# skywoodsz/qm_control

Hardware: NVIDIA H100
Metric: mpc_wbc_iters_per_s (higher is better)
Workload: dtype f64

## Files before the change

### qm_control_b200/csrc/kernels/mpc_api.cuh

```cuda
#pragma once
#include <cuda_runtime.h>

#include <string>
#include <vector>

#include "dev_common.cuh"

namespace qmb {

constexpr int EMAX = 32, KMAX = 4, TARGET_DIM = 37;
constexpr int LDX = 36, LDB = 28, LDG = 34, LDH = 24;
constexpr int ST_AR = 0;
constexpr int ST_BR = ST_AR + 9 * LDX;
constexpr int ST_Q = ST_BR + 9 * LDB;
constexpr int Q_PACKED = 480;
__host__ __device__ constexpr int q_row_offset(int r) { return (r & 1) ? 2 * ((r >> 1) + 1) * ((r >> 1) + 1) : 2 * (r >> 1) * ((r >> 1) + 1); }
__host__ __device__ constexpr int q_row_padded(int r) { return (r + 2) & ~1; }
static_assert(q_row_offset(29) + q_row_padded(29) == Q_PACKED && q_row_offset(1) == 2 && q_row_offset(2) == 4 && q_row_offset(3) == 8, "packed lower triangle with even rows");
constexpr int ST_TAIL = ST_Q + Q_PACKED;
constexpr int T_PXJ = 0;
constexpr int T_b = 144, T_q = 174, T_r = 204;
constexpr int T_RT = 222;
constexpr int T_SJ = 276;
constexpr int T_PU2 = 372, T_PED = 380;
constexpr int T_MISC = 396;
constexpr int T_INT = 400;
constexpr int TAIL_DBL = 428, STAGE_DBL = ST_TAIL + TAIL_DBL;
constexpr int SI_TYPE = 0, SI_M = 1, SI_NDEP = 2, SI_DEP = 3, SI_FREE = 19, SI_PIV = 37, SI_PCOL = 41;
static_assert(STAGE_DBL == 1484 && (ST_BR % 2 == 0) && (ST_Q % 2 == 0) && (ST_TAIL % 2 == 0) && (TAIL_DBL % 2 == 0), "16-byte aligned pieces");
constexpr int GAIN_DBL = 18 * LDG;
constexpr int ROBOT_DBL = 8;

struct MpcSolutionDev { int32_t* n_nodes = nullptr; double* t = nullptr; int32_t* event = nullptr; double* x = nullptr; double* u = nullptr; };

struct MpcBuffers {
  int B = 0, nmax = 0, cur = 0;
  double *t0 = nullptr, *x0 = nullptr, *event_times = nullptr, *target_times = nullptr, *target_states = nullptr;
  int32_t *n_events = nullptr, *modes = nullptr, *n_target = nullptr;
  MpcSolutionDev sol[2];
  double *ddp_trial = nullptr;
  double *node_rec = nullptr;
  double *stage = nullptr, *gains = nullptr, *dx = nullptr, *du = nullptr, *robot = nullptr, *step_info = nullptr;
  int32_t *stage_i = nullptr, *status = nullptr;
};
bool mpc_alloc(MpcBuffers& m, int B, int nmax, std::string& err, std::vector<void*>& allocs, cudaStream_t stream);
int mpc_configure_device();

struct MpcProblemDev { const double* t0; const double* x0; const int32_t* n_events; const double* event_times; const int32_t* modes; const int32_t* n_target; const double* target_times; const double* target_states;
                       const double* srbd; const double* tuning; };

int mpc_solve_launch(const DevModel* mdl, const DevModel& host_mdl, MpcBuffers& m, const MpcProblemDev& p, int b0, int b1, cudaStream_t stream, cudaEvent_t* ev = nullptr);
double measure_fp64_peak(cudaStream_t stream);
// ... 5 lines not shown
```

### qm_control_b200/csrc/kernels/mpc_kernels.cu

```cuda
#include <cstdlib>
#include "mpc_api.cuh"
#include "mpc_device.cuh"
#include "node_eval.cuh"
#include "wlinalg.cuh"

namespace qmb {

#ifndef QMB_LQ_WARPS
#define QMB_LQ_WARPS 4
#endif
#ifndef QMB_LQ_MINB
#define QMB_LQ_MINB 4
#endif
constexpr int LQ_WARPS = QMB_LQ_WARPS, LS_WARPS = 4, SETUP_WARPS = 4;
enum { MST_ITER_CAP = 1, MST_OVERFLOW = 2, MST_NAN = 4, MST_NOT_PD = 8, MST_NO_STEP = 16, MST_CONVERGED = 32, MST_NEG_DT = 64 };

__device__ __forceinline__ double interval_start(double t, int ev) { return ev == 2 ? t + WEAK_EPS : t; }
__device__ __forceinline__ double interval_end(double t, int ev) { return ev == 1 ? t - WEAK_EPS : t; }
__device__ __forceinline__ int clamp_events(int ne) { return ne < 0 ? 0 : (ne > EMAX ? EMAX : ne); }
__device__ __forceinline__ int clamp_targets(int nk) { return nk < 1 ? 1 : (nk > KMAX ? KMAX : nk); }
__device__ __forceinline__ int flag_mask(int mode) { int m = 0; for (int i = 0; i < 4; ++i) if (contact_flag(mode, i)) m |= 1 << i; return m; }

struct SetupIdx { int iu, ix; double au, ax; };
__host__ __device__ inline size_t setup_smem_per_warp(int nmax) { return (size_t)nmax * (8 + 8 + 4 + sizeof(SetupIdx) + 4) + 8 * EMAX + 64; }
__global__ void __launch_bounds__(32 * SETUP_WARPS) mpc_setup_kernel(const DevModel* __restrict__ mdl, int b0, int B, int nmax, MpcProblemDev p, MpcSolutionDev prev, MpcSolutionDev next, int32_t* __restrict__ status) {
  const int warp = threadIdx.x >> 5, lane = threadIdx.x & 31; const int b = b0 + blockIdx.x * SETUP_WARPS + warp; if (b >= B) return;
  extern __shared__ __align__(16) unsigned char s_setup[];
  unsigned char* base = s_setup + (size_t)warp * ((setup_smem_per_warp(nmax) + 15) & ~(size_t)15);
  double* spt = reinterpret_cast<double*>(base); double* sgt = spt + nmax; SetupIdx* sidx = reinterpret_cast<SetupIdx*>(sgt + nmax); double* sev = reinterpret_cast<double*>(sidx + nmax);
  int32_t* sge = reinterpret_cast<int32_t*>(sev + EMAX); int32_t* sflag = sge + nmax; unsigned char* smodes = reinterpret_cast<unsigned char*>(sflag + nmax);
  const double t0 = p.t0[b], tf = t0 + mdl->time_horizon, dt = mdl->dt; const int ne = clamp_events(p.n_events[b]); int st = 0;
  if (ne != p.n_events[b] || clamp_targets(p.n_target[b]) != p.n_target[b]) st |= MST_OVERFLOW;
  { const double* gev = p.event_times + (size_t)b * EMAX; const int32_t* gmodes = p.modes + (size_t)b * (EMAX + 1); sev[lane] = (lane < ne) ? gev[lane] : 0.0; smodes[lane] = (unsigned char)((lane <= ne) ? gmodes[lane] : 15); if (lane == 0) smodes[EMAX] = (unsigned char)((EMAX <= ne) ? gmodes[EMAX] : 15); }
  __syncwarp();
  const double* ev = sev; const unsigned char* modes = smodes;
// ... 36 lines not shown
  for (int k = 0; k < n - 1; ++k) {
    const int flag = sflag[k]; const SetupIdx ix = sidx[k]; double uk = 0.0;
    if (flag == 1) { uk = lerp(pu, ix.iu, ix.au); xk = lerp(px, ix.ix, ix.ax); }
    else if (flag == 0) { const int mode = ix.iu; int nst = 0; for (int i = 0; i < 4; ++i) nst += contact_flag(mode, i); if (lane < 12 && (lane % 3) == 2 && contact_flag(mode, lane / 3)) uk = srbd_of(mdl, p.srbd, b)->m * 9.81 / nst; }
    if (lane < NX) { gu[(size_t)k * NU + lane] = uk; gx[(size_t)(k + 1) * NX + lane] = xk; }
  }
  if (lane < NX && n >= 1) gu[(size_t)(n - 1) * NU + lane] = 0.0;
  if (lane == 0) status[b] = st;
}

struct LqLate { double BrdF[9 * 12], BrdJ[3 * NJ], bvec[NX]; };
struct alignas(16) LqSmem {
  ne::NodeRec rec;
  QuadWs quad; LegWs leg[4];
  double x[NX], u[NU];
  double Rw[NU][3];
  double Pe_full[NU], rs[NU];
  double ev[EMAX];
  int dep_idx[MAXDEP], free_idx[MU], col_of_input[NU];
  unsigned char modes[EMAX + 1];
};
static_assert(sizeof(LqLate) <= 4 * sizeof(ne::FootBlk) && offsetof(ne::NodeRec, foot) == 0, "LqLate overlays the foot blocks of the record");
static_assert(sizeof(LqSmem) % 16 == 0 && offsetof(LqSmem, rec) == 0, "aligned record slice");
static_assert((sizeof(LqSmem) * LQ_WARPS + 1024) * QMB_LQ_MINB <= 232448, "projection kernel: QMB_LQ_MINB CTAs of LQ_WARPS warps per SM (10.0 KB per node: four CTAs of four warps = 16 nodes in flight; 20 warps would fit the shared memory, not the 96-register budget)");

#ifndef QMB_FL_MINB
#define QMB_FL_MINB 2
#endif
constexpr int FL_WARPS = 4, FL_TILE = ne::EE_DBL;
constexpr int FL_UROW = NU + 1;
constexpr int FL_SMEM = FL_WARPS * 32 * (FL_TILE + 1 + FL_UROW) * 8;
__global__ void __launch_bounds__(32 * FL_WARPS, QMB_FL_MINB) mpc_flow_kernel(const DevModel* __restrict__ mdl, int b0, int B, int nmax, MpcProblemDev p, MpcSolutionDev sol, double* __restrict__ rec, const int32_t* __restrict__ status) {
  extern __shared__ __align__(16) unsigned char smem_raw[]; double (*tile)[32][FL_TILE + 1] = reinterpret_cast<double (*)[32][FL_TILE + 1]>(smem_raw);
  const int tid = threadIdx.x, warp = tid >> 5, lane = tid & 31; const long long gid = (long long)blockIdx.x * (32 * FL_WARPS) + tid;
  const int b = b0 + (int)(gid / nmax), k = (int)(gid % nmax);
  const int n = (b < B) ? sol.n_nodes[b] : 0;
  bool work = b < B && k < n && !(status[b] & MST_CONVERGED);
  const bool terminal = work && (k == n - 1);
  if (work && !terminal && sol.event[(size_t)b * nmax + k] == 1) work = false;
  const unsigned active = __ballot_sync(FULL, work); if (!active) return;
  const SrbdConst* sc = srbd_of(mdl, p.srbd, work ? b : b0);
  double* row = &tile[warp][lane][0]; double* gbase = rec + ((size_t)b0 * nmax + (size_t)(gid - lane)) * ne::NODE_REC_DBL;
  auto flush = [&](int off, int cnt) {
    __syncwarp();
#pragma unroll 4
    for (int rw = 0; rw < 32; ++rw) if ((active >> rw) & 1u) { double* g = gbase + (size_t)rw * ne::NODE_REC_DBL + off;
#pragma unroll
// ... 86 lines not shown
  if (!terminal && ek == 1) {
    double* tl = sg + ST_TAIL; int32_t* si = reinterpret_cast<int32_t*>(tl + T_INT);
    double d = 0.0; if (lane < NX) { d = xv - xnv; tl[T_b + lane] = d; }
    const double ss = warp_sum(d * d);
    if (lane == 0) { si[SI_TYPE] = 1; si[SI_M] = 0; si[SI_NDEP] = 0; tl[T_MISC] = 0.0; tl[T_MISC + 1] = 0.0; tl[T_MISC + 2] = ss; tl[T_MISC + 3] = 0.0; }
    return;
  }
  { double2* rs = reinterpret_cast<double2*>(&sm.rec);
#pragma unroll
    for (int q = 0; q < (ne::NODE_REC_DBL / 2 + 31) / 32; ++q) { const int e = lane + 32 * q; if (e < ne::NODE_REC_DBL / 2) rs[e] = rr[q]; } }
  __syncwarp();
  const int lfp = pack_leg_foot(mdl);
  const int nk = clamp_targets(p.n_target[b]); const double* tt = p.target_times + (size_t)b * KMAX; const double* ts = p.target_states + (size_t)b * KMAX * TARGET_DIM;
  const double t = interval_start(tk, ek);
  const double dt = terminal ? 0.0 : interval_end(tk1, ek1) - t;
  const int mode = mode_at_time(ev, modes, ne, t); const int fm = terminal ? 0 : flag_mask(mode);
  if (!terminal && !(dt > 0.0) && lane == 0) atomicOr(&status[b], MST_NEG_DT);
  double cost_val = 0.0, eq_ss = 0.0; int ndep = 0, m = 0; double b1v[3] = {0.0, 0.0, 0.0}, b2v[3] = {0.0, 0.0, 0.0}, a1[9], a2[9];
  {
  struct XU { double x[NX], u[NU]; }; static_assert(offsetof(LqSmem, u) == offsetof(LqSmem, x) + NX * 8, "x then u");
  cost_val = stage_cost_quad(mdl, sc, tuning_of(mdl, TUNED ? p.tuning : nullptr, b), reinterpret_cast<const XU*>(sm.x), &sm.rec.ee, &sm.quad, target_xnom(tt, ts, nk, t, lane), fm, terminal, lane);
  if (terminal) {
    double* tl = sg + ST_TAIL; int32_t* si = reinterpret_cast<int32_t*>(tl + T_INT);
    for (int r = 0; r < NX; ++r) { const int a = ee_pos(r); if (lane < q_row_padded(r)) { const int cc = (lane <= r) ? ee_pos(lane) : -1; sg[ST_Q + q_row_offset(r) + lane] = (a >= 0 && cc >= 0) ? sm.quad.E[a * 12 + cc] : 0.0; } }
    if (lane < NX) tl[T_q + lane] = sm.quad.qf[lane];
    if (lane == 0) { si[SI_TYPE] = 2; si[SI_M] = 0; si[SI_NDEP] = 0; tl[T_MISC] = 0.0; tl[T_MISC + 1] = cost_val; tl[T_MISC + 2] = 0.0; tl[T_MISC + 3] = 0.0; }
    return;
  }
  int nd_before = 0; for (int i = 0; i < 4; ++i) if (i < lane) nd_before += ((fm >> i) & 1) ? 3 : 4;
  ndep = 0; for (int i = 0; i < 4; ++i) ndep += ((fm >> i) & 1) ? 3 : 4;
  m = NU - ndep;
  for (int e = lane; e < NU * 3; e += 32) { const int i = e / 3, c = e - 3 * i; sm.Rw[i][c] = (i < 24) ? quad_R(mdl, &sm.quad, i, 3 * (i / 3) + c) : (c == 0 ? quad_R(mdl, &sm.quad, i, i) : 0.0); }
  bool swing_ok = true; int pivot = -1;
  if (lane < 4) {
    const int i = lane; const int first = mdl->foot_leg[i]; LegWs& L = sm.leg[i]; L.first = first; L.stance = (fm >> i) & 1;
    if (L.stance) { for (int j = 0; j < 3; ++j) { sm.dep_idx[nd_before + j] = 12 + first + j; L.dep[j] = 1; } L.pivot = -1; for (int a = 0; a < 3; ++a) eq_ss += sm.rec.foot[i].e[a] * sm.rec.foot[i].e[a]; }
    else {
      double zp, zv; swing_ok = swing_reference(mdl, ev, modes, ne, i, t, zp, zv);
      double ez = sm.rec.foot[i].e[2] - zv; if (mdl->position_error_gain != 0.0) ez += mdl->position_error_gain * (sm.rec.foot[i].pf[2] - zp);
      sm.rec.foot[i].e[2] = ez;
      for (int a = 0; a < 3; ++a) { sm.dep_idx[nd_before + a] = 3 * i + a; eq_ss += sm.u[3 * i + a] * sm.u[3 * i + a]; }
      eq_ss += ez * ez;
      double best = -1.0; for (int j = 0; j < 3; ++j) { const double a = fabs(sm.rec.foot[i].Jl[3 * j + 2]); if (a > best) { best = a; pivot = j; } }
      sm.dep_idx[nd_before + 3] = 12 + first + pivot; L.pivot = pivot; for (int j = 0; j < 3; ++j) L.dep[j] = (j == pivot);
    }
  }
  eq_ss = warp_sum(eq_ss);
// ... 86 lines not shown
        if (pos >= 0) { double acc = 0.0;
          for (int j = 0; j < 3; ++j) if (L.dep[j]) acc = fma(lt.BrdJ[rr * NJ + first + j], L.Px[j][pos], acc);
          v += acc; } }
      out[rr] = v;
    }
#pragma unroll
    for (int rr = 0; rr < 9; ++rr) { if (c == rr + 3) out[rr] += 1.0; sg[ST_AR + rr * LDX + c] = out[rr]; }
  } else if (lane == 31) {
#pragma unroll
    for (int rr = 0; rr < 9; ++rr) sg[ST_AR + rr * LDX + 31] = 0.0;
  }
  for (int e = lane; e < 36; e += 32) sg[ST_AR + (e >> 2) * LDX + 32 + (e & 3)] = 0.0;
  for (int e = lane; e < 144; e += 32) { const int j12 = e / 12, c = e - 12 * j12; const LegWs& L = sm.leg[foot_of_leg_joint(lfp, j12)]; const int j = j12 % 3; tl[T_PXJ + e] = L.dep[j] ? L.Px[j][c] : 0.0; }
  for (int e = lane; e < 9 * LDB; e += 32) {
    const int rr = e / LDB, a = e - rr * LDB; const int r = 3 + rr; double v = 0.0;
    if (a < m) { const int fa = sm.free_idx[a];
      if (fa < 12) v = lt.BrdF[rr * 12 + fa];
      else if (r < 6) { v = lt.BrdJ[rr * NJ + fa - 12];
        if (fa < 24) { const LegWs& L = sm.leg[foot_of_leg_joint(lfp, fa - 12)]; if (!L.stance) { const int jf = (fa - 12) % 3; v += lt.BrdJ[rr * NJ + L.first + L.pivot] * L.Pu2[jf > L.pivot ? jf - 1 : jf]; } } }
    }
    sg[ST_BR + e] = v;
  }
  if (lane < NX) {
    const int r = lane; double acc[NX];
    if (mdl->q_is_diag) { const double qrr = mdl->Qdiag[r];
#pragma unroll
      for (int c = 0; c < NX; ++c) acc[c] = (c == r) ? qrr : 0.0; }
    else {
#pragma unroll
      for (int c = 0; c < NX; ++c) acc[c] = mdl->Q[r * NX + c]; }
    double qv = sm.quad.qf[r];
    const int ea = ee_pos(r);
    if (ea >= 0) {
#pragma unroll
      for (int c = 0; c < 6; ++c) { acc[6 + c] += sm.quad.E[ea * 12 + c]; acc[24 + c] += sm.quad.E[ea * 12 + 6 + c]; }
    }
#pragma unroll
    for (int i = 0; i < 4; ++i) {
      const LegWs& L = sm.leg[i]; const int first = L.first;
      const int pr = (r < 6) ? r : ((r >= 9 && r < 12) ? r - 3 : ((r >= 12 + first && r < 15 + first) ? 9 + r - 12 - first : -1));
      if (pr >= 0) {
        double blk[12];
#pragma unroll
        for (int c = 0; c < 12; ++c) blk[c] = 0.0;
        double w3[3] = {0.0, 0.0, 0.0};
        for (int j = 0; j < 3; ++j) if (L.dep[j]) { const double pj = L.Px[j][pr]; qv = fma(pj, sm.rs[12 + first + j], qv);
#pragma unroll
          for (int a = 0; a < 3; ++a) w3[a] = fma(pj, sm.Rw[12 + first + j][a], w3[a]); }
        for (int a = 0; a < 3; ++a) if (L.dep[a]) { const double wa = w3[a];
#pragma unroll
          for (int c = 0; c < 12; ++c) blk[c] = fma(wa, L.Px[a][c], blk[c]); }
#pragma unroll
        for (int c = 0; c < 6; ++c) acc[c] += blk[c];
#pragma unroll
        for (int c = 0; c < 3; ++c) acc[9 + c] += blk[6 + c];
#pragma unroll
        for (int l = 0; l < 4; ++l) if (first == 3 * l) {
#pragma unroll
          for (int c = 0; c < 3; ++c) acc[12 + 3 * l + c] += blk[9 + c]; }
      }
    }
    const double dq = sm.quad.qdiag[r];
#pragma unroll
    for (int c = 0; c < NX; ++c) if (r <= c) sg[ST_Q + q_row_offset(c) + r] = dt * (acc[c] + ((c == r) ? dq : 0.0));
    if (!(r & 1)) sg[ST_Q + q_row_offset(r) + r + 1] = 0.0;
    tl[T_q + r] = dt * qv;
  }
  for (int e = lane; e < 8 * 12; e += 32) tl[T_SJ + e] = 0.0;
  __syncwarp();
  if (lane < MU) {
    const int a = lane; double rt[3] = {0.0, 0.0, 0.0}; double rtil = 0.0;
    if (a < m) {
      const int fa = sm.free_idx[a]; double rv = sm.rs[fa]; int li = -1, jf = -1;
      if (fa >= 12 && fa < 24) { li = foot_of_leg_joint(lfp, fa - 12); jf = (fa - 12) % 3; }
      const bool swing_joint = li >= 0 && !sm.leg[li].stance;
      const double* Rl = sm.Rw[jf >= 0 ? fa - jf : 0];
      if (swing_joint) {
        const LegWs& L = sm.leg[li]; const int pv = L.pivot; const int jfi = jf > pv ? jf - 1 : jf; const double pu = L.Pu2[jfi];
        rv += pu * sm.rs[fa - jf + pv];
        const double coef = Rl[3 * jf + pv]; double* Srow = tl + T_SJ + (2 * li + jfi) * 12;
        const double cf = dt * (coef + pu * Rl[3 * pv + pv]);
        for (int c = 0; c < 12; ++c) Srow[c] = cf * L.Px[pv][c];
      }
      rtil = dt * rv;
      if (fa >= 24) rt[0] = dt * sm.Rw[fa][0];
      else { const int bi = fa / 3;
        for (int jc = 0; jc < 3; ++jc) { const int fc = 3 * bi + jc; if (sm.col_of_input[fc] < 0) continue;
          double v = sm.Rw[fa][jc];
          if (swing_joint) { const LegWs& L = sm.leg[li]; const int pv = L.pivot; const double pa = L.Pu2[jf > pv ? jf - 1 : jf], pc = L.Pu2[jc > pv ? jc - 1 : jc];
            v += pa * Rl[3 * pv + jc] + Rl[3 * jf + pv] * pc + pa * Rl[3 * pv + pv] * pc; }
          rt[jc] = dt * v; } }
    }
    tl[T_r + a] = rtil; tl[T_RT + 3 * a] = rt[0]; tl[T_RT + 3 * a + 1] = rt[1]; tl[T_RT + 3 * a + 2] = rt[2];
  }
  if (lane < 4) { const LegWs& L = sm.leg[lane]; tl[T_PU2 + 2 * lane] = L.Pu2[0]; tl[T_PU2 + 2 * lane + 1] = L.Pu2[1]; si[SI_PIV + lane] = L.stance ? -1 : L.pivot;
    int nf = 0; for (int jj = 0; jj < 3; ++jj) if (!L.stance && jj != L.pivot) si[SI_PCOL + 2 * lane + nf++] = L.free_col[jj]; if (L.stance) { si[SI_PCOL + 2 * lane] = -1; si[SI_PCOL + 2 * lane + 1] = -1; } }
  if (lane < MAXDEP) { const int d = lane; double pe = 0.0; int di = -1; if (d < ndep) { di = sm.dep_idx[d]; pe = sm.Pe_full[di]; } tl[T_PED + d] = pe; si[SI_DEP + d] = di; }
  if (lane < MU) si[SI_FREE + lane] = (lane < m) ? sm.free_idx[lane] : -1;
  if (lane == 0) { si[SI_TYPE] = 0; si[SI_M] = m; si[SI_NDEP] = ndep; tl[T_MISC] = dtw; tl[T_MISC + 1] = dt * cost_val; tl[T_MISC + 2] = dt * dyn_ss; tl[T_MISC + 3] = dt * eq_ss; }
}

#ifndef QMB_TMA
#define QMB_TMA 1
#endif
constexpr int RIC_THREADS = 128, RIC_NTYPE = 512;
struct RicSmem {
  double P[NX * LDX];
  double A[NX * LDX];
  double W[NX * LDX];
  double Bm[NX * LDB], PB[NX * LDB];
  double G[MU * LDG];
  double H[MU * LDH];
  double Lt[MU * MU];
  alignas(16) double tail[TAIL_DBL];
  double dx[32], dut[32], tmp[32];
  double red[RIC_THREADS / 32][4];
  alignas(8) unsigned long long bar[4];
  int flag; int pad_;
  signed char srow[MU + 2], sfirst[MU + 2];
  unsigned char ntype[RIC_NTYPE];
};
static_assert(sizeof(RicSmem) <= 57344 - 64, "Riccati kernel must keep four CTAs per SM");

__device__ __forceinline__ unsigned smem_u32(const void* p) { return (unsigned)__cvta_generic_to_shared(p); }
__device__ __forceinline__ void mbar_init(unsigned long long* b, unsigned count) { asm volatile("mbarrier.init.shared::cta.b64 [%0], %1;\n" ::"r"(smem_u32(b)), "r"(count) : "memory"); }
__device__ __forceinline__ void mbar_expect_tx(unsigned long long* b, unsigned bytes) { asm volatile("mbarrier.arrive.expect_tx.shared::cta.b64 _, [%0], %1;\n" ::"r"(smem_u32(b)), "r"(bytes) : "memory"); }
__device__ __forceinline__ void mbar_wait(unsigned long long* b, unsigned parity) {
  asm volatile("{\n .reg .pred p;\n WAIT_LOOP:\n mbarrier.try_wait.parity.shared::cta.b64 p, [%0], %1;\n @p bra WAIT_DONE;\n bra WAIT_LOOP;\n WAIT_DONE:\n}\n" ::"r"(smem_u32(b)), "r"(parity) : "memory");
}
__device__ __forceinline__ void bulk_g2s(void* dst, const void* src, unsigned bytes, unsigned long long* bar) {
  asm volatile("cp.async.bulk.shared::cluster.global.mbarrier::complete_tx::bytes [%0], [%1], %2, [%3];\n" ::"r"(smem_u32(dst)), "l"(src), "r"(bytes), "r"(smem_u32(bar)) : "memory");
}
__device__ __forceinline__ int fresh_tid() { int t; asm volatile("mov.u32 %0, %%tid.x;" : "=r"(t)); return t; }
__device__ __forceinline__ void cp_async16(void* smem_dst, const void* gmem_src) { asm volatile("cp.async.cg.shared.global [%0], [%1], 16;\n" ::"r"(smem_u32(smem_dst)), "l"(gmem_src) : "memory"); }
__device__ __forceinline__ void cp_async_wait_all() { asm volatile("cp.async.wait_all;\n" ::: "memory"); }
struct CopyGroup {
  unsigned long long* bar; unsigned phase;
  __device__ __forceinline__ void begin(unsigned bytes, int tid) { if (QMB_TMA && tid == 0) mbar_expect_tx(bar, bytes); }
  __device__ __forceinline__ void copy(void* dst, const void* src, unsigned bytes, int tid, int nthr = RIC_THREADS, int t0 = 0) {
    if (QMB_TMA) { if (tid == 0) bulk_g2s(dst, src, bytes, bar); }
// ... 17 lines not shown
#pragma unroll
    for (int n = 0; n < NT; ++n) bf[n] = ok ? Y[kr * ldy + j0 + 8 * n + g] : 0.0;
#pragma unroll
    for (int m = 0; m < MT; ++m)
#pragma unroll
      for (int n = 0; n < NT; ++n) dmma884(c[m][n], a[m], bf[n]);
  }
}
template <int MT, int NT>
__device__ __forceinline__ void cfrag_load(const double* M, int ld, int i0, int j0, int rows, double (&c)[MT][NT][2], int g, int t) {
#pragma unroll
  for (int m = 0; m < MT; ++m)
#pragma unroll
    for (int n = 0; n < NT; ++n) { const int ri = i0 + 8 * m + g;
      if (ri < rows) { const double2 v = *reinterpret_cast<const double2*>(M + ri * ld + j0 + 8 * n + 2 * t); c[m][n][0] = v.x; c[m][n][1] = v.y; } else { c[m][n][0] = 0.0; c[m][n][1] = 0.0; } }
}
template <int MT, int NT>
__device__ __forceinline__ void cfrag_store(double* M, int ld, int i0, int j0, int rows, const double (&c)[MT][NT][2], int g, int t) {
#pragma unroll
  for (int m = 0; m < MT; ++m)
#pragma unroll
    for (int n = 0; n < NT; ++n) { const int ri = i0 + 8 * m + g; if (ri < rows) *reinterpret_cast<double2*>(M + ri * ld + j0 + 8 * n + 2 * t) = make_double2(c[m][n][0], c[m][n][1]); }
}
__device__ __forceinline__ int sup_pos(int j, int first) { return j < 6 ? j : ((j >= 9 && j < 12) ? j - 3 : (((unsigned)(j - 12 - first) < 3u) ? 9 + j - 12 - first : -1)); }

__global__ void __launch_bounds__(RIC_THREADS, 4) mpc_riccati_kernel(const DevModel* __restrict__ mdl, int b0, int B, int nmax, MpcProblemDev p, MpcSolutionDev sol, const double* __restrict__ stage,
                                                                  double* __restrict__ gains, double* __restrict__ dxo, double* __restrict__ duo, double* __restrict__ robot, int32_t* __restrict__ status) {
  extern __shared__ __align__(16) unsigned char smem_raw[];
  RicSmem& sm = *reinterpret_cast<RicSmem*>(smem_raw);
  const int tid = threadIdx.x, warp = tid >> 5, lane = tid & 31, ti = tid >> 2, jb = tid & 3; const int b = b0 + blockIdx.x;
  if (status[b] & MST_CONVERGED) return;
  const int n = sol.n_nodes[b]; const int N = n - 1;
  const double* sgb = stage + (size_t)b * nmax * STAGE_DBL; double* gb = gains + (size_t)b * nmax * GAIN_DBL;
  const int lfp = pack_leg_foot(mdl); const double imass = 1.0 / srbd_of(mdl, p.srbd, b)->m;
  for (int e = tid; e < (int)(sizeof(RicSmem) / 8); e += RIC_THREADS) reinterpret_cast<double*>(&sm)[e] = 0.0;
  __syncthreads();
  if (tid < NX && (tid < 3 || tid >= 24)) sm.A[tid * LDX + tid] = 1.0;
  if (tid == 0) { for (int i = 0; i < 4; ++i) mbar_init(&sm.bar[i], 1); asm volatile("fence.mbarrier_init.release.cluster;\n" ::: "memory"); }
  asm volatile("fence.proxy.async.shared::cta;\n" ::: "memory");
  const bool types_in_smem = n <= RIC_NTYPE;
  auto rec_type = [&](int k) -> int { return reinterpret_cast<const int32_t*>(sgb + (size_t)k * STAGE_DBL + ST_TAIL + T_INT)[SI_TYPE]; };
  if (types_in_smem) for (int k = tid; k < n; k += RIC_THREADS) sm.ntype[k] = (unsigned char)rec_type(k);
  auto node_type = [&](int k) -> int { return types_in_smem ? (int)sm.ntype[k] : rec_type(k); };
  CopyGroup gAB{&sm.bar[0], 0u}, gT{&sm.bar[1], 0u}, gQ{&sm.bar[2], 0u}, gF1{&sm.bar[3], 0u};
  auto issue_ab = [&](int k) { const double* sg = sgb + (size_t)k * STAGE_DBL; gAB.begin((9 * LDX + 9 * LDB) * 8, tid);
    gAB.copy(sm.A + 3 * LDX, sg + ST_AR, 9 * LDX * 8, tid); gAB.copy(sm.Bm + 3 * LDB, sg + ST_BR, 9 * LDB * 8, tid); };
  auto issue_tail = [&](int k) { gT.begin(TAIL_DBL * 8, tid); gT.copy(sm.tail, sgb + (size_t)k * STAGE_DBL + ST_TAIL, TAIL_DBL * 8, tid); };
  auto issue_q = [&](int k) { gQ.begin(Q_PACKED * 8, tid); gQ.copy(sm.Bm, sgb + (size_t)k * STAGE_DBL + ST_Q, Q_PACKED * 8, tid); };
  auto expand = [&]() { const int tid = fresh_tid();
    const double* tl = sm.tail; const int32_t* si = reinterpret_cast<const int32_t*>(tl + T_INT); const double dtw = tl[T_MISC];
    for (int e = tid; e < 144; e += RIC_THREADS) { const int j12 = e / 12, c = e - 12 * j12; const int col = sup_col(c, 3 * (j12 / 3));
      sm.A[(12 + j12) * LDX + col] = ((col == 12 + j12) ? 1.0 : 0.0) + dtw * tl[T_PXJ + e]; }
    if (tid < NX && (tid < 3 || tid >= 12)) sm.A[tid * LDX + NX] = tl[T_b + tid];
    for (int e = tid; e < 21 * MU; e += RIC_THREADS) {
      const int rr = e / MU, a = e - rr * MU; const int r = rr < 3 ? rr : rr + 9; const int fa = si[SI_FREE + a]; double v = 0.0;
      if (fa >= 0) {
        if (r < 3) { if (fa < 12 && fa - 3 * (fa / 3) == r) v = dtw * imass; }
        else if (fa == r) v = dtw;
        else if (fa >= 12 && fa < 24) { const int j = fa - 12, lg = j / 3, foot = (lfp >> (2 * lg)) & 3; const int pv = si[SI_PIV + foot];
          if (pv >= 0 && r == 12 + 3 * lg + pv) { const int jf = j - 3 * lg; v = dtw * tl[T_PU2 + 2 * foot + (jf > pv ? jf - 1 : jf)]; } }
      }
      sm.Bm[r * LDB + a] = v;
    }
    if (tid < MU) { const int fa = si[SI_FREE + tid]; int slot = -1, first = 0;
      if (fa >= 12 && fa < 24) { const int j = fa - 12, lg = j / 3, foot = (lfp >> (2 * lg)) & 3; const int pv = si[SI_PIV + foot]; if (pv >= 0) { const int jf = j - 3 * lg; slot = 2 * foot + (jf > pv ? jf - 1 : jf); first = 3 * lg; } }
      sm.srow[tid] = (signed char)slot; sm.sfirst[tid] = (signed char)first; }
  };
  for (int e = tid; e < NX * NX; e += RIC_THREADS) { const int r = e / NX, c = e - r * NX; sm.P[r * LDX + c] = sgb[(size_t)N * STAGE_DBL + ST_Q + q_row_offset(r > c ? r : c) + (r > c ? c : r)]; }
  if (tid < NX) sm.P[tid * LDX + NX] = sgb[(size_t)N * STAGE_DBL + ST_TAIL + T_q + tid];
  double perf0 = 0, perf1 = 0, perf2 = 0;
  for (int k = tid; k < n; k += RIC_THREADS) { const double* pf = sgb + (size_t)k * STAGE_DBL + ST_TAIL + T_MISC + 1; perf0 += pf[0]; perf1 += pf[1]; perf2 += pf[2]; }
  if (tid < NX) { const double d = p.x0[(size_t)b * NX + tid] - sol.x[(size_t)b * nmax * NX + tid]; sm.dx[tid] = d; perf1 += d * d; }
  perf0 = warp_sum(perf0); perf1 = warp_sum(perf1); perf2 = warp_sum(perf2);
  if (lane == 0) { sm.red[warp][0] = perf0; sm.red[warp][1] = perf1; sm.red[warp][2] = perf2; }
  __syncthreads();
  double perf[3]; for (int i = 0; i < 3; ++i) perf[i] = sm.red[0][i] + sm.red[1][i] + sm.red[2][i] + sm.red[3][i];
  if (N >= 1) { issue_tail(N - 1); if (node_type(N - 1) != 1) issue_ab(N - 1); gT.wait(); if (node_type(N - 1) != 1) expand(); }
  int st = 0;
  const int g = lane >> 2, t = lane & 3;
  for (int k = N - 1; k >= 0; --k) {
    const int type = node_type(k); const int tnext = k > 0 ? node_type(k - 1) : 1;
    if (type == 1) {
      __syncthreads();
      if (tid < NX) { double sv = sm.P[tid * LDX + NX]; for (int j = 0; j < NX; ++j) sv = fma(sm.P[tid * LDX + j], sm.tail[T_b + j], sv); sm.tmp[tid] = sv; }
      __syncthreads();
      if (tid < NX) sm.P[tid * LDX + NX] = sm.tmp[tid];
      if (k > 0) { issue_tail(k - 1); if (tnext != 1) issue_ab(k - 1); gT.wait(); if (tnext != 1) expand(); }
      continue;
    }
    gAB.wait(); if (QMB_TMA) __syncthreads();
    const double dtw_k = sm.tail[T_MISC]; const int acol0 = reinterpret_cast<const int32_t*>(sm.tail + T_INT)[SI_M] - 6;
// ... 20 lines not shown
    if (tid < NX) sm.P[tid * LDX + NX] = sm.tail[T_q + tid];
    { const double* tl = sm.tail; const int32_t* si = reinterpret_cast<const int32_t*>(tl + T_INT); const int mm = si[SI_M];
      double c[3][1][2];
#pragma unroll
      for (int mt = 0; mt < 3; ++mt) { const int a = 8 * mt + g; const bool rowok = a < MU; const int slot = rowok ? sm.srow[a] : -1, first = rowok ? sm.sfirst[a] : 0;
#pragma unroll
        for (int e = 0; e < 2; ++e) { const int j = 8 * warp + 2 * t + e; double v = 0.0;
          if (rowok) { if (j == NX) v = tl[T_r + a]; else if (slot >= 0 && j < NX) { const int ps = sup_pos(j, first); if (ps >= 0) v = tl[T_SJ + slot * 12 + ps]; }
            if ((unsigned)(a - acol0) < 6u) v = fma(dtw_k, sm.W[(24 + a - acol0) * LDX + j], v); }
          c[mt][0][e] = v; } }
      warp_mma<24, 3, 1, false>(sm.Bm, LDB, 0, sm.W, LDX, 8 * warp, c, g, t); cfrag_store<3, 1>(sm.G, LDG, 0, 8 * warp, MU, c, g, t);
      if (warp < 3) { double d[3][1][2];
#pragma unroll
        for (int mt = 0; mt < 3; ++mt) { const int a = 8 * mt + g; const int fa = (a < MU) ? si[SI_FREE + a] : -1;
#pragma unroll
          for (int e = 0; e < 2; ++e) { const int cc = 8 * warp + 2 * t + e; double v = 0.0;
            if (a < MU && cc < MU) { if (a >= mm) v = (a == cc) ? 1.0 : 0.0;
              else if (fa >= 24) v = (a == cc) ? tl[T_RT + 3 * a] : 0.0;
              else { const int fc = si[SI_FREE + cc]; if (fc >= 0 && fc / 3 == fa / 3) v = tl[T_RT + 3 * a + fc - 3 * (fc / 3)]; }
              if ((unsigned)(a - acol0) < 6u) v = fma(dtw_k, sm.PB[(24 + a - acol0) * LDB + cc], v); }
            d[mt][0][e] = v; } }
        warp_mma<24, 3, 1, false>(sm.Bm, LDB, 0, sm.PB, LDB, 8 * warp, d, g, t); cfrag_store<3, 1>(sm.H, LDH, 0, 8 * warp, MU, d, g, t); } }
    __syncthreads();
    issue_q(k);
    if (k > 0) issue_tail(k - 1);
    const int sw = (k + b) & 3;
    if (!QMB_TMA) gQ.wait();
    if (warp == sw) {
      if (QMB_TMA) gQ.skip();
      double hr[MU], y[MU]; double dinv = 0.0; bool ok = true; double* Yb = sm.PB;
#pragma unroll
      for (int c = 0; c < MU; ++c) { hr[c] = (lane < MU) ? sm.H[c * LDH + lane] : 0.0; y[c] = sm.G[c * LDG + lane]; }
#pragma unroll
      for (int j = 0; j < MU; ++j) {
        const double djj = __shfl_sync(FULL, hr[j], j); if (!(djj > 0.0)) ok = false;
        const double inv = rsqrt(djj); const double lij = hr[j] * inv;
        if (lane == j) dinv = inv;
        if (lane < MU) sm.Lt[j * MU + lane] = lij;
        y[j] *= inv; Yb[j * LDX + lane] = y[j];
#pragma unroll
        for (int c = j + 1; c < MU; ++c) { const double lcj = __shfl_sync(FULL, lij, c); hr[c] = fma(-lij, lcj, hr[c]); y[c] = fma(-lcj, y[j], y[c]); }
      }
      if (lane < MU) sm.dut[lane] = dinv;
      if (!ok && lane == 0) sm.flag = 1;
      __syncwarp();
      double* gk = gb + (size_t)k * GAIN_DBL;
#pragma unroll
      for (int a = MU - 1; a >= 0; --a) {
        asm volatile("" ::: "memory");
        y[a] *= sm.dut[a];
        gk[a * LDG + lane] = -y[a];
#pragma unroll
        for (int c = 0; c < a; ++c) y[c] = fma(-sm.Lt[c * MU + a], y[a], y[c]);
      }
    } else {
      if (QMB_TMA) gQ.wait();
      const int hi = (warp - sw - 1) & 3;
      for (int tile = hi; tile < 16; tile += 3) { const int i0 = 8 * (tile >> 2), j0 = 8 * (tile & 3);
        double c[1][1][2]; const int ri = i0 + g;
#pragma unroll
        for (int e = 0; e < 2; ++e) { const int cj = j0 + 2 * t + e; double v = (ri < NX && cj <= NX) ? (cj == NX ? sm.P[ri * LDX + NX] : (cj <= ri ? sm.Bm[q_row_offset(ri) + cj] : sm.Bm[q_row_offset(cj) + ri])) : 0.0;
          if (ri >= 24 && ri < NX && cj <= NX) v += sm.W[ri * LDX + cj];
          c[0][0][e] = v; }
        warp_mma<24, 1, 1, false>(sm.A, LDX, i0, sm.W, LDX, j0, c, g, t); cfrag_store<1, 1>(sm.P, LDX, i0, j0, NX, c, g, t); }
    }
    __syncthreads();
    if (sm.flag) { st |= MST_NOT_PD; if (k > 0) gT.wait(); break; }
    if (k > 0) { if (tnext != 1) issue_ab(k - 1); gT.wait(); if (tnext != 1) expand(); }
    { const double* Yb = sm.PB; const int i0 = 16 * (warp >> 1), j0 = 16 * (warp & 1);
      double c[2][2][2]; cfrag_load<2, 2>(sm.P, LDX, i0, j0, NX, c, g, t); warp_mma<MU, 2, 2, true>(Yb, LDX, i0, Yb, LDX, j0, c, g, t); cfrag_store<2, 2>(sm.P, LDX, i0, j0, NX, c, g, t); }
  }
  __syncthreads();
  double armijo = 0.0, dxn2 = 0.0, dun2 = 0.0;
  if (!(st & MST_NOT_PD)) {
    auto issue_fwd = [&](int k) {
      if (k >= N) return; const double* sg = sgb + (size_t)k * STAGE_DBL; const bool ev = node_type(k) == 1;
      auto issue = [&](CopyGroup& cg, double* kb, double* ab, double* bb) {
        cg.begin((ev ? 0 : (GAIN_DBL + 9 * LDX + 9 * LDB) * 8) + TAIL_DBL * 8, tid);
        cg.copy(ab + 9 * LDX, sg + ST_TAIL, TAIL_DBL * 8, tid);
        if (!ev) { cg.copy(kb, gb + (size_t)k * GAIN_DBL, GAIN_DBL * 8, tid); cg.copy(ab, sg + ST_AR, 9 * LDX * 8, tid); cg.copy(bb, sg + ST_BR, 9 * LDB * 8, tid); } };
      if (k & 1) issue(gF1, sm.W, sm.P, sm.PB); else issue(gAB, sm.G, sm.A, sm.Bm); };
    issue_fwd(0);
    for (int k = 0; k < N; ++k) {
      const int o = k & 1; const double* Kb = o ? sm.W : sm.G; const double* ARb = o ? sm.P : sm.A; const double* BRb = o ? sm.PB : sm.Bm; const double* tl = (o ? sm.P : sm.A) + 9 * LDX;
      double* dxk = dxo + ((size_t)b * nmax + k) * NX; double* duk = duo + ((size_t)b * nmax + k) * NU;
      const double* dxc = (k & 1) ? sm.tmp : sm.dx; double* dxn = (k & 1) ? sm.dx : sm.tmp;
// ... 394 lines not shown
```

### qm_control_b200/csrc/kernels/mpc_scalar.cuh

```cuda
#pragma once
#include "dev_common.cuh"

namespace qmb {

constexpr int MU = 18;
constexpr int MAXDEP = 16;
constexpr double WEAK_EPS = 1e-6;
QMB_HD int pack_leg_foot(const DevModel* __restrict__ mdl) { return mdl->leg_foot[0] | (mdl->leg_foot[1] << 2) | (mdl->leg_foot[2] << 4) | (mdl->leg_foot[3] << 6); }
QMB_HD int foot_of_leg_joint(int lfp, int j) { return (lfp >> (2 * (j / 3))) & 3; }
QMB_HD int lower_bound_idx(const double* a, int n, double t) { int lo = 0, hi = n; while (lo < hi) { const int mid = (lo + hi) >> 1; if (a[mid] < t) lo = mid + 1; else hi = mid; } return lo; }
template <class MT> QMB_HD int mode_at_time(const double* ev, const MT* modes, int ne, double t) { return modes[lower_bound_idx(ev, ne, t)]; }
QMB_HD void time_segment(const double* times, int n, double t, int& index, double& alpha) {
  if (n <= 1) { index = 0; alpha = 1.0; return; }
  const int part = lower_bound_idx(times, n, t); int idx = (part != 0 || t != times[0]) ? part - 1 : 0; const int last = n - 1;
  if (idx >= 0) {
    if (idx < last) { const double len = times[idx + 1] - times[idx], till = times[idx + 1] - t; index = idx; alpha = (len > 2.0 * 2.220446049250313e-16) ? till / len : (till > 0.5 * len ? 1.0 : 0.0); return; }
    index = (last - 1 > 0) ? last - 1 : 0; alpha = 0.0; return;
  }
  index = 0; alpha = 1.0;
}
template <class MT> QMB_HD bool swing_reference(const DevModel* __restrict__ mdl, const double* ev, const MT* modes, int ne, int leg, double t, double& zp, double& zv) {
  const int np = ne + 1; const int p = lower_bound_idx(ev, ne, t); zp = 0.0; zv = 0.0;
  if (contact_flag(modes[p], leg)) return true;
  int start = -1; for (int ip = p - 1; ip >= 0; --ip) if (contact_flag(modes[ip], leg)) { start = ip; break; }
  int fin = np - 1; for (int ip = p + 1; ip < np; ++ip) if (contact_flag(modes[ip], leg)) { fin = ip - 1; break; }
  if (start < 0 || fin >= np - 1) return false;
  const double t0 = ev[start], t1 = ev[fin]; const double scaling = fmin(1.0, (t1 - t0) / mdl->swing_time_scale); const double tm = 0.5 * (t0 + t1), zm = scaling * mdl->swing_height;
  double ta, pa, va, tb, pb, vb;
  if (t < tm) { ta = t0; pa = 0.0; va = scaling * mdl->lift_off_velocity; tb = tm; pb = zm; vb = 0.0; } else { ta = tm; pa = zm; va = 0.0; tb = t1; pb = 0.0; vb = scaling * mdl->touch_down_velocity; }
  const double dtt = tb - ta, dp = pb - pa, dv = vb - va; const double c0 = pa, c1 = va * dtt, c2 = -(3.0 * va + dv) * dtt + 3.0 * dp, c3 = (2.0 * va + dv) * dtt - 2.0 * dp; const double idt = 1.0 / dtt, tn = (t - ta) * idt;
  zp = ((c3 * tn + c2) * tn + c1) * tn + c0; zv = ((3.0 * c3 * tn + 2.0 * c2) * tn + c1) * idt; return true;
}
QMB_HD void relaxed_barrier(double mu, double delta, double h, double& p0, double& p1, double& p2) {
  const bool inside = h > delta; const double lg = log(inside ? h : delta);
  if (inside) { const double ih = 1.0 / h; p0 = -mu * lg; p1 = -mu * ih; p2 = mu * ih * ih; }
  else { const double t = (h - 2.0 * delta) / delta; p0 = mu * (-lg + 0.5 * t * t - 0.5); p1 = mu * (h - 2.0 * delta) / (delta * delta); p2 = mu / (delta * delta); }
}

QMB_HD int ee_pos(int c) { return (c >= 6 && c < 12) ? c - 6 : (c >= 24 ? c - 18 : -1); }
QMB_HD int ee_col(int i) { return i < 6 ? 6 + i : 18 + i; }
QMB_HD int sup_col(int pos, int first) { return pos < 6 ? pos : (pos < 9 ? pos + 3 : 12 + first + pos - 9); }

struct QuadWs { double E[144], fric[36], qdiag[NX], rdiag[NU], qf[NX], rf[NU]; };
QMB_HD double quad_R(const DevModel* __restrict__ mdl, const QuadWs* q, int i, int j) {
  if (i >= 24 || j >= 24) return (i == j) ? mdl->Rarm[i - 24] + q->rdiag[i] : 0.0;
  const int bi = i / 3; if (bi != j / 3) return 0.0;
  double v = mdl->Rblk[bi][(i - 3 * bi) * 3 + (j - 3 * bi)]; if (i == j) v += q->rdiag[i]; if (i < 12) v += q->fric[bi * 9 + (i - 3 * bi) * 3 + (j - 3 * bi)]; return v; }
struct LegWs {
  double Px[3][12];
  double G[9];
  double Pu2[2];
  int dep[3];
  int pivot, stance, first, free_col[3];
};

}
```

Measured before the change: 24.51.

## Store factored stage cost instead of packed dense Q and rebuild Q in Riccati

Replaces the packed 30x30 lower-triangle Q in each stage record with a compact cost block: the triangle of the 12x12 end-effector block, the diagonal, the leg Rw terms and a flag for a dense model Q. The Riccati kernel now pulls this block together with A/B in one TMA group and rebuilds Q on the fly, adding the leg projection term with an extra small MMA. This shrinks the stage record, removes the separate Q copy and its barrier, and drops the per-lane dense Q assembly from the LQ kernel. It also raises LQ occupancy (min blocks 5) and halves the node-type table. The cost is extra index arithmetic and a named barrier among three warps in the Riccati inner loop.

Result: faster. 24.94, median of 6 (+1.8%).

```diff
diff --git a/qm_control_b200/csrc/kernels/mpc_api.cuh b/qm_control_b200/csrc/kernels/mpc_api.cuh
--- a/qm_control_b200/csrc/kernels/mpc_api.cuh
+++ b/qm_control_b200/csrc/kernels/mpc_api.cuh
@@ -12,12 +12,15 @@
 constexpr int LDX = 36, LDB = 28, LDG = 34, LDH = 24;
 constexpr int ST_AR = 0;
 constexpr int ST_BR = ST_AR + 9 * LDX;
-constexpr int ST_Q = ST_BR + 9 * LDB;
-constexpr int Q_PACKED = 480;
-__host__ __device__ constexpr int q_row_offset(int r) { return (r & 1) ? 2 * ((r >> 1) + 1) * ((r >> 1) + 1) : 2 * (r >> 1) * ((r >> 1) + 1); }
-__host__ __device__ constexpr int q_row_padded(int r) { return (r + 2) & ~1; }
-static_assert(q_row_offset(29) + q_row_padded(29) == Q_PACKED && q_row_offset(1) == 2 && q_row_offset(2) == 4 && q_row_offset(3) == 8, "packed lower triangle with even rows");
-constexpr int ST_TAIL = ST_Q + Q_PACKED;
+constexpr int ST_C = ST_BR + 9 * LDB;
+constexpr int C_E = 0;
+constexpr int C_D = 78;
+constexpr int C_RL = 108;
+constexpr int C_DQ = 144;
+constexpr int COST_DBL = 146;
+__host__ __device__ constexpr int e_tri(int i, int j) { return i * (i + 1) / 2 + j; }
+static_assert(e_tri(11, 11) + 1 == C_D && C_D + 30 == C_RL && C_RL + 36 == C_DQ, "cost block");
+constexpr int ST_TAIL = ST_C + COST_DBL;
 constexpr int T_PXJ = 0;
 constexpr int T_b = 144, T_q = 174, T_r = 204;
 constexpr int T_RT = 222;
@@ -27,7 +30,7 @@
 constexpr int T_INT = 400;
 constexpr int TAIL_DBL = 428, STAGE_DBL = ST_TAIL + TAIL_DBL;
 constexpr int SI_TYPE = 0, SI_M = 1, SI_NDEP = 2, SI_DEP = 3, SI_FREE = 19, SI_PIV = 37, SI_PCOL = 41;
-static_assert(STAGE_DBL == 1484 && (ST_BR % 2 == 0) && (ST_Q % 2 == 0) && (ST_TAIL % 2 == 0) && (TAIL_DBL % 2 == 0), "16-byte aligned pieces");
+static_assert(STAGE_DBL == 1150 && (ST_BR % 2 == 0) && (ST_C % 2 == 0) && (ST_TAIL % 2 == 0) && (TAIL_DBL % 2 == 0) && T_PXJ == 0, "16-byte aligned pieces, Px rows behind the cost block");
 constexpr int GAIN_DBL = 18 * LDG;
 constexpr int ROBOT_DBL = 8;
 
diff --git a/qm_control_b200/csrc/kernels/mpc_kernels.cu b/qm_control_b200/csrc/kernels/mpc_kernels.cu
--- a/qm_control_b200/csrc/kernels/mpc_kernels.cu
+++ b/qm_control_b200/csrc/kernels/mpc_kernels.cu
@@ -10,7 +10,7 @@
 #define QMB_LQ_WARPS 4
 #endif
 #ifndef QMB_LQ_MINB
-#define QMB_LQ_MINB 4
+#define QMB_LQ_MINB 5
 #endif
 constexpr int LQ_WARPS = QMB_LQ_WARPS, LS_WARPS = 4, SETUP_WARPS = 4;
 enum { MST_ITER_CAP = 1, MST_OVERFLOW = 2, MST_NAN = 4, MST_NOT_PD = 8, MST_NO_STEP = 16, MST_CONVERGED = 32, MST_NEG_DT = 64 };
@@ -93,7 +93,7 @@
 };
 static_assert(sizeof(LqLate) <= 4 * sizeof(ne::FootBlk) && offsetof(ne::NodeRec, foot) == 0, "LqLate overlays the foot blocks of the record");
 static_assert(sizeof(LqSmem) % 16 == 0 && offsetof(LqSmem, rec) == 0, "aligned record slice");
-static_assert((sizeof(LqSmem) * LQ_WARPS + 1024) * QMB_LQ_MINB <= 232448, "projection kernel: QMB_LQ_MINB CTAs of LQ_WARPS warps per SM (10.0 KB per node: four CTAs of four warps = 16 nodes in flight; 20 warps would fit the shared memory, not the 96-register budget)");
+static_assert((sizeof(LqSmem) * LQ_WARPS + 1024) * QMB_LQ_MINB <= 232448, "projection kernel: QMB_LQ_MINB CTAs of LQ_WARPS warps per SM (10.0 KB per node: 20 warps = 20 nodes in flight at 96 registers)");
 
 #ifndef QMB_FL_MINB
 #define QMB_FL_MINB 2
@@ -226,7 +226,7 @@
   cost_val = stage_cost_quad(mdl, sc, tuning_of(mdl, TUNED ? p.tuning : nullptr, b), reinterpret_cast<const XU*>(sm.x), &sm.rec.ee, &sm.quad, target_xnom(tt, ts, nk, t, lane), fm, terminal, lane);
   if (terminal) {
     double* tl = sg + ST_TAIL; int32_t* si = reinterpret_cast<int32_t*>(tl + T_INT);
-    for (int r = 0; r < NX; ++r) { const int a = ee_pos(r); if (lane < q_row_padded(r)) { const int cc = (lane <= r) ? ee_pos(lane) : -1; sg[ST_Q + q_row_offset(r) + lane] = (a >= 0 && cc >= 0) ? sm.quad.E[a * 12 + cc] : 0.0; } }
+    for (int e = lane; e < 144; e += 32) { const int i = e / 12, j = e - 12 * i; if (j <= i) sg[ST_C + C_E + e_tri(i, j)] = sm.quad.E[e]; }
     if (lane < NX) tl[T_q + lane] = sm.quad.qf[lane];
     if (lane == 0) { si[SI_TYPE] = 2; si[SI_M] = 0; si[SI_NDEP] = 0; tl[T_MISC] = 0.0; tl[T_MISC + 1] = cost_val; tl[T_MISC + 2] = 0.0; tl[T_MISC + 3] = 0.0; }
     return;
@@ -359,50 +359,17 @@
     sg[ST_BR + e] = v;
   }
   if (lane < NX) {
-    const int r = lane; double acc[NX];
-    if (mdl->q_is_diag) { const double qrr = mdl->Qdiag[r];
-#pragma unroll
-      for (int c = 0; c < NX; ++c) acc[c] = (c == r) ? qrr : 0.0; }
-    else {
-#pragma unroll
-      for (int c = 0; c < NX; ++c) acc[c] = mdl->Q[r * NX + c]; }
-    double qv = sm.quad.qf[r];
-    const int ea = ee_pos(r);
-    if (ea >= 0) {
-#pragma unroll
-      for (int c = 0; c < 6; ++c) { acc[6 + c] += sm.quad.E[ea * 12 + c]; acc[24 + c] += sm.quad.E[ea * 12 + 6 + c]; }
-    }
-#pragma unroll
+    const int r = lane; double qv = sm.quad.qf[r];
     for (int i = 0; i < 4; ++i) {
-      const LegWs& L = sm.leg[i]; const int first = L.first;
-      const int pr = (r < 6) ? r : ((r >= 9 && r < 12) ? r - 3 : ((r >= 12 + first && r < 15 + first) ? 9 + r - 12 - first : -1));
-      if (pr >= 0) {
-        double blk[12];
-#pragma unroll
-        for (int c = 0; c < 12; ++c) blk[c] = 0.0;
-        double w3[3] = {0.0, 0.0, 0.0};
-        for (int j = 0; j < 3; ++j) if (L.dep[j]) { const double pj = L.Px[j][pr]; qv = fma(pj, sm.rs[12 + first + j], qv);
-#pragma unroll
-          for (int a = 0; a < 3; ++a) w3[a] = fma(pj, sm.Rw[12 + first + j][a], w3[a]); }
-        for (int a = 0; a < 3; ++a) if (L.dep[a]) { const double wa = w3[a];
-#pragma unroll
-          for (int c = 0; c < 12; ++c) blk[c] = fma(wa, L.Px[a][c], blk[c]); }
-#pragma unroll
-        for (int c = 0; c < 6; ++c) acc[c] += blk[c];
-#pragma unroll
-        for (int c = 0; c < 3; ++c) acc[9 + c] += blk[6 + c];
-#pragma unroll
-        for (int l = 0; l < 4; ++l) if (first == 3 * l) {
-#pragma unroll
-          for (int c = 0; c < 3; ++c) acc[12 + 3 * l + c] += blk[9 + c]; }
-      }
-    }
-    const double dq = sm.quad.qdiag[r];
-#pragma unroll
-    for (int c = 0; c < NX; ++c) if (r <= c) sg[ST_Q + q_row_offset(c) + r] = dt * (acc[c] + ((c == r) ? dq : 0.0));
-    if (!(r & 1)) sg[ST_Q + q_row_offset(r) + r + 1] = 0.0;
+      const LegWs& L = sm.leg[i]; const int first = L.first; const int pr = sup_pos(r, first);
+      if (pr >= 0) for (int j = 0; j < 3; ++j) if (L.dep[j]) qv = fma(L.Px[j][pr], sm.rs[12 + first + j], qv);
+    }
     tl[T_q + r] = dt * qv;
-  }
+    sg[ST_C + C_D + r] = dt * (mdl->Qdiag[r] + sm.quad.qdiag[r]);
+  }
+  for (int e = lane; e < 144; e += 32) { const int i = e / 12, j = e - 12 * i; if (j <= i) sg[ST_C + C_E + e_tri(i, j)] = dt * sm.quad.E[e]; }
+  for (int e = lane; e < 36; e += 32) { const int lg = e / 9, j = (e - 9 * lg) / 3, a = e - 9 * lg - 3 * j; sg[ST_C + C_RL + e] = dt * sm.Rw[12 + 3 * lg + j][a]; }
+  if (lane < 2) sg[ST_C + C_DQ + lane] = (lane == 0 && !mdl->q_is_diag) ? dt : 0.0;
   for (int e = lane; e < 8 * 12; e += 32) tl[T_SJ + e] = 0.0;
   __syncwarp();
   if (lane < MU) {
@@ -440,7 +407,7 @@
 #ifndef QMB_TMA
 #define QMB_TMA 1
 #endif
-constexpr int RIC_THREADS = 128, RIC_NTYPE = 512;
+constexpr int RIC_THREADS = 128, RIC_NTYPE = 256;
 struct RicSmem {
   double P[NX * LDX];
   double A[NX * LDX];
@@ -450,9 +417,10 @@
   double H[MU * LDH];
   double Lt[MU * MU];
   alignas(16) double tail[TAIL_DBL];
+  alignas(16) double cost[COST_DBL + 144];
   double dx[32], dut[32], tmp[32];
   double red[RIC_THREADS / 32][4];
-  alignas(8) unsigned long long bar[4];
+  alignas(8) unsigned long long bar[3];
   int flag; int pad_;
   signed char srow[MU + 2], sfirst[MU + 2];
   unsigned char ntype[RIC_NTYPE];
@@ -516,8 +484,6 @@
 #pragma unroll
     for (int n = 0; n < NT; ++n) { const int ri = i0 + 8 * m + g; if (ri < rows) *reinterpret_cast<double2*>(M + ri * ld + j0 + 8 * n + 2 * t) = make_double2(c[m][n][0], c[m][n][1]); }
 }
-__device__ __forceinline__ int sup_pos(int j, int first) { return j < 6 ? j : ((j >= 9 && j < 12) ? j - 3 : (((unsigned)(j - 12 - first) < 3u) ? 9 + j - 12 - first : -1)); }
-
 __global__ void __launch_bounds__(RIC_THREADS, 4) mpc_riccati_kernel(const DevModel* __restrict__ mdl, int b0, int B, int nmax, MpcProblemDev p, MpcSolutionDev sol, const double* __restrict__ stage,
                                                                   double* __restrict__ gains, double* __restrict__ dxo, double* __restrict__ duo, double* __restrict__ robot, int32_t* __restrict__ status) {
   extern __shared__ __align__(16) unsigned char smem_raw[];
@@ -530,17 +496,19 @@
   for (int e = tid; e < (int)(sizeof(RicSmem) / 8); e += RIC_THREADS) reinterpret_cast<double*>(&sm)[e] = 0.0;
   __syncthreads();
   if (tid < NX && (tid < 3 || tid >= 24)) sm.A[tid * LDX + tid] = 1.0;
-  if (tid == 0) { for (int i = 0; i < 4; ++i) mbar_init(&sm.bar[i], 1); asm volatile("fence.mbarrier_init.release.cluster;\n" ::: "memory"); }
+  if (tid == 0) { for (int i = 0; i < 3; ++i) mbar_init(&sm.bar[i], 1); asm volatile("fence.mbarrier_init.release.cluster;\n" ::: "memory"); }
   asm volatile("fence.proxy.async.shared::cta;\n" ::: "memory");
   const bool types_in_smem = n <= RIC_NTYPE;
   auto rec_type = [&](int k) -> int { return reinterpret_cast<const int32_t*>(sgb + (size_t)k * STAGE_DBL + ST_TAIL + T_INT)[SI_TYPE]; };
   if (types_in_smem) for (int k = tid; k < n; k += RIC_THREADS) sm.ntype[k] = (unsigned char)rec_type(k);
   auto node_type = [&](int k) -> int { return types_in_smem ? (int)sm.ntype[k] : rec_type(k); };
-  CopyGroup gAB{&sm.bar[0], 0u}, gT{&sm.bar[1], 0u}, gQ{&sm.bar[2], 0u}, gF1{&sm.bar[3], 0u};
-  auto issue_ab = [&](int k) { const double* sg = sgb + (size_t)k * STAGE_DBL; gAB.begin((9 * LDX + 9 * LDB) * 8, tid);
-    gAB.copy(sm.A + 3 * LDX, sg + ST_AR, 9 * LDX * 8, tid); gAB.copy(sm.Bm + 3 * LDB, sg + ST_BR, 9 * LDB * 8, tid); };
+  CopyGroup gAB{&sm.bar[0], 0u}, gT{&sm.bar[1], 0u}, gF1{&sm.bar[2], 0u};
+  constexpr int QC_DBL = COST_DBL + 144;
+  auto issue_ab = [&](int k) { const double* sg = sgb + (size_t)k * STAGE_DBL; gAB.begin((9 * LDX + 9 * LDB + QC_DBL) * 8, tid);
+    gAB.copy(sm.A + 3 * LDX, sg + ST_AR, 9 * LDX * 8, tid); gAB.copy(sm.Bm + 3 * LDB, sg + ST_BR, 9 * LDB * 8, tid); gAB.copy(sm.cost, sg + ST_C, QC_DBL * 8, tid); };
   auto issue_tail = [&](int k) { gT.begin(TAIL_DBL * 8, tid); gT.copy(sm.tail, sgb + (size_t)k * STAGE_DBL + ST_TAIL, TAIL_DBL * 8, tid); };
-  auto issue_q = [&](int k) { gQ.begin(Q_PACKED * 8, tid); gQ.copy(sm.Bm, sgb + (size_t)k * STAGE_DBL + ST_Q, Q_PACKED * 8, tid); };
+  constexpr int QC_RPD = 12 * LDB;
+  static_assert(2 * QC_RPD <= NX * LDB, "leg-term operands fit the B~ buffer");
   auto expand = [&]() { const int tid = fresh_tid();
     const double* tl = sm.tail; const int32_t* si = reinterpret_cast<const int32_t*>(tl + T_INT); const double dtw = tl[T_MISC];
     for (int e = tid; e < 144; e += RIC_THREADS) { const int j12 = e / 12, c = e - 12 * j12; const int col = sup_col(c, 3 * (j12 / 3));
@@ -560,7 +528,8 @@
       if (fa >= 12 && fa < 24) { const int j = fa - 12, lg = j / 3, foot = (lfp >> (2 * lg)) & 3; const int pv = si[SI_PIV + foot]; if (pv >= 0) { const int jf = j - 3 * lg; slot = 2 * foot + (jf > pv ? jf - 1 : jf); first = 3 * lg; } }
       sm.srow[tid] = (signed char)slot; sm.sfirst[tid] = (signed char)first; }
   };
-  for (int e = tid; e < NX * NX; e += RIC_THREADS) { const int r = e / NX, c = e - r * NX; sm.P[r * LDX + c] = sgb[(size_t)N * STAGE_DBL + ST_Q + q_row_offset(r > c ? r : c) + (r > c ? c : r)]; }
+  for (int e = tid; e < NX * NX; e += RIC_THREADS) { const int r = e / NX, c = e - r * NX; const int a = ee_pos(r), cc = ee_pos(c);
+    sm.P[r * LDX + c] = (a >= 0 && cc >= 0) ? sgb[(size_t)N * STAGE_DBL + ST_C + C_E + (a > cc ? e_tri(a, cc) : e_tri(cc, a))] : 0.0; }
   if (tid < NX) sm.P[tid * LDX + NX] = sgb[(size_t)N * STAGE_DBL + ST_TAIL + T_q + tid];
   double perf0 = 0, perf1 = 0, perf2 = 0;
   for (int k = tid; k < n; k += RIC_THREADS) { const double* pf = sgb + (size_t)k * STAGE_DBL + ST_TAIL + T_MISC + 1; perf0 += pf[0]; perf1 += pf[1]; perf2 += pf[2]; }
@@ -627,12 +596,9 @@
             d[mt][0][e] = v; } }
         warp_mma<24, 3, 1, false>(sm.Bm, LDB, 0, sm.PB, LDB, 8 * warp, d, g, t); cfrag_store<3, 1>(sm.H, LDH, 0, 8 * warp, MU, d, g, t); } }
     __syncthreads();
-    issue_q(k);
     if (k > 0) issue_tail(k - 1);
     const int sw = (k + b) & 3;
-    if (!QMB_TMA) gQ.wait();
     if (warp == sw) {
-      if (QMB_TMA) gQ.skip();
       double hr[MU], y[MU]; double dinv = 0.0; bool ok = true; double* Yb = sm.PB;
 #pragma unroll
       for (int c = 0; c < MU; ++c) { hr[c] = (lane < MU) ? sm.H[c * LDH + lane] : 0.0; y[c] = sm.G[c * LDG + lane]; }
@@ -659,14 +625,25 @@
         for (int c = 0; c < a; ++c) y[c] = fma(-sm.Lt[c * MU + a], y[a], y[c]);
       }
     } else {
-      if (QMB_TMA) gQ.wait();
       const int hi = (warp - sw - 1) & 3;
+      const double* cb = sm.cost;
+      for (int e = 32 * hi + lane; e < 12 * 24; e += 96) { const int k = e / 24, col = e - 24 * k, lg = k / 3, j = k - 3 * lg; const int ps = sup_pos(col, 3 * lg);
+        double pv = 0.0, rv = 0.0;
+        if (ps >= 0) { const double* pa = cb + COST_DBL + 36 * lg + ps; const double* rl = cb + C_RL + 9 * lg + 3 * j; pv = pa[12 * j]; rv = fma(rl[0], pa[0], fma(rl[1], pa[12], rl[2] * pa[24])); }
+        sm.Bm[k * LDB + col] = pv; sm.Bm[QC_RPD + k * LDB + col] = rv; }
+      asm volatile("fence.proxy.async.shared::cta;\n" ::: "memory");
+      asm volatile("bar.sync 1, 96;" ::: "memory");
       for (int tile = hi; tile < 16; tile += 3) { const int i0 = 8 * (tile >> 2), j0 = 8 * (tile & 3);
         double c[1][1][2]; const int ri = i0 + g;
 #pragma unroll
-        for (int e = 0; e < 2; ++e) { const int cj = j0 + 2 * t + e; double v = (ri < NX && cj <= NX) ? (cj == NX ? sm.P[ri * LDX + NX] : (cj <= ri ? sm.Bm[q_row_offset(ri) + cj] : sm.Bm[q_row_offset(cj) + ri])) : 0.0;
+        for (int e = 0; e < 2; ++e) { const int cj = j0 + 2 * t + e; double v = 0.0;
+          if (ri < NX && cj < NX) {
+            if (cj == ri) v = cb[C_D + ri]; else { const double dq = cb[C_DQ]; if (dq != 0.0) v = dq * mdl->Q[ri * NX + cj]; }
+            if (i0 != 16 && j0 != 16) { const int a = ee_pos(ri), ac = ee_pos(cj); if (a >= 0 && ac >= 0) v += cb[C_E + (a > ac ? e_tri(a, ac) : e_tri(ac, a))]; }
+          } else if (ri < NX && cj == NX) v = sm.P[ri * LDX + NX];
           if (ri >= 24 && ri < NX && cj <= NX) v += sm.W[ri * LDX + cj];
           c[0][0][e] = v; }
+        if (i0 < 24 && j0 < 24) warp_mma<12, 1, 1, false>(sm.Bm, LDB, i0, sm.Bm + QC_RPD, LDB, j0, c, g, t);
         warp_mma<24, 1, 1, false>(sm.A, LDX, i0, sm.W, LDX, j0, c, g, t); cfrag_store<1, 1>(sm.P, LDX, i0, j0, NX, c, g, t); }
     }
     __syncthreads();
diff --git a/qm_control_b200/csrc/kernels/mpc_scalar.cuh b/qm_control_b200/csrc/kernels/mpc_scalar.cuh
--- a/qm_control_b200/csrc/kernels/mpc_scalar.cuh
+++ b/qm_control_b200/csrc/kernels/mpc_scalar.cuh
@@ -40,6 +40,7 @@
 QMB_HD int ee_pos(int c) { return (c >= 6 && c < 12) ? c - 6 : (c >= 24 ? c - 18 : -1); }
 QMB_HD int ee_col(int i) { return i < 6 ? 6 + i : 18 + i; }
 QMB_HD int sup_col(int pos, int first) { return pos < 6 ? pos : (pos < 9 ? pos + 3 : 12 + first + pos - 9); }
+QMB_HD int sup_pos(int j, int first) { return j < 6 ? j : ((j >= 9 && j < 12) ? j - 3 : (((unsigned)(j - 12 - first) < 3u) ? 9 + j - 12 - first : -1)); }
 
 struct QuadWs { double E[144], fric[36], qdiag[NX], rdiag[NU], qf[NX], rf[NU]; };
 QMB_HD double quad_R(const DevModel* __restrict__ mdl, const QuadWs* q, int i, int j) {
```
